# simplify23/TPS_PP

Hardware: AMD Instinct MI355X
Metric: rectified images/sec (3x32x100) (higher is better)
Workload: dtype f32; 1 GPU; BASELINE.json configs[1]: fused TPS grid-gen + bilinear grid_sample HIP kernel, batch 512 per GPU, 3x32x100 fp32, 20 fiducials, inputs resident in HBM; batch_per_gpu=512, rotating_buffer_sets=14, streams=3, repeats=1

## Files before the change

### tps_pp_amd/csrc/tpspp_warp_pair.h

```cpp
#pragma once
#include "tpspp_warp_dev.h"

namespace tpspp_pair {

using namespace tpspp_dev;

typedef float v4f __attribute__((ext_vector_type(4)));
typedef float v4f_a4 __attribute__((ext_vector_type(4), aligned(4)));
typedef __attribute__((address_space(1))) char gchar;

struct PairParams {
    const float* in; const float* ctrl; const float* inv_delta_c;
    const float* packed;
    const float* p_hat;
    int p_hat_ld;
    int N;
    float* out; float* grid; int32_t* idx;
    int zero_off;
    int out_off;
    long long* trace;
};

template <int F>
__device__ __forceinline__ constexpr int perm_y(int k) { return (k + F / 2) % F; }
template <int F>
__device__ __forceinline__ constexpr int perm_x(int k) { return k < F / 2 ? F / 2 - 1 - k : F + F / 2 - 1 - k; }

__device__ __forceinline__ void store16_nt(gchar* p, v4f v)
{
    asm volatile("global_store_dwordx4 %0, %1, off nt\n\ts_nop 1" ::"v"(p), "v"(v) : "memory");
}

__device__ __forceinline__ void wait_flag(const float* flag_word, int want)
{
    const volatile int* f = reinterpret_cast<const volatile int*>(flag_word);
    while (*f < want) __builtin_amdgcn_s_sleep(1);
}
__device__ __forceinline__ void wait_flag_lds(const float* flag_word, int want)
{
    typedef __attribute__((address_space(3))) const volatile int lds_cvint;
    lds_cvint* f = (lds_cvint*)(size_t)(unsigned)(size_t)flag_word;
    while (__builtin_amdgcn_readfirstlane(*f) < want) __builtin_amdgcn_s_sleep(1);
}

template <int OFF>
__device__ __forceinline__ void flag_add(unsigned addr, int one)
{
    asm volatile("ds_add_u32 %0, %1 offset:%2" ::"v"(addr), "v"(one), "n"(OFF) : "memory");
}

struct TapsLite {
    int o00;
    float nw, ne, sw, se;
    float wx, wy;
    bool inx, iny;
    int x0, y0;
};
__device__ __forceinline__ TapsLite make_taps_lite(float gx, float gy, int H, int W)
{
    TapsLite t;
    const float limx = (float)(W - 1), limy = (float)(H - 1);
    float ix = (gx + 1.0f) * (0.5f * limx);
    float iy = (gy + 1.0f) * (0.5f * limy);
    ix = (ix > 0.0f) ? ix : 0.0f;
    iy = (iy > 0.0f) ? iy : 0.0f;
    ix = __builtin_fminf(ix, limx);
    iy = __builtin_fminf(iy, limy);
    const float w = __builtin_amdgcn_fractf(ix), nn = __builtin_amdgcn_fractf(iy);
    int x0, y0;
    asm("v_cvt_flr_i32_f32 %0, %1" : "=v"(x0) : "v"(ix));
    asm("v_cvt_flr_i32_f32 %0, %1" : "=v"(y0) : "v"(iy));
    const float e = 1.0f - w, s = 1.0f - nn;
    t.nw = s * e; t.ne = s * w; t.sw = nn * e; t.se = nn * w;
    t.wx = w; t.wy = nn;
    t.inx = ix < limx;
    t.iny = iy < limy;
    t.o00 = __mul24(y0, W) + x0;
    t.x0 = x0; t.y0 = y0;
    return t;
}

constexpr int kPairFlags = 4;
constexpr int kPairLoaders = 3;
constexpr int kPairAwait = 6;
constexpr int kPairKB = 4;

constexpr int kPairVarPacked = 1;
constexpr int kPairVarMfma = 2;
typedef float v2f __attribute__((ext_vector_type(2)));

template <int OH, int OW>
struct PairGeo {
    static constexpr int halfW = OW / 2;
    static constexpr int PW = (halfW + 3) & ~3;
    static constexpr int CGP = PW / 4;
    static constexpr int CG = (halfW - 2) / 4;
    static constexpr int SC0 = CG * 4;
    static constexpr int SW = OW - 2 * SC0;
    static constexpr int nthr = (OH / 2) * CG * 4;
    static constexpr int NW = nthr / kWave;
    static_assert(OW % 4 == 0 && (OH / 2) % 8 == 0 && nthr % kWave == 0, "needs whole 4 x 8 pixel blocks, whole wavefronts");
    static_assert(SW == 4 && OH * SW == 2 * kWave, "the centre strip is 4 columns, two wavefronts per image");
    static_assert(NW % 4 == 0 && NW >= 4, "the compute wavefronts spread evenly over the four SIMDs");
};
__host__ __device__ inline void pair_thread_pixel(int t, int CG, int* r, int* c)
{
    const int hw = t >> 5, l5 = t & 31, rg = hw / CG, cg = hw - rg * CG;
    *r = rg * 8 + (l5 >> 2);
    *c = cg * 4 + (l5 & 3);
}

template <int F, int C, int HC, int WC, int OH, int OW, bool AUX, bool TRACE, int VAR = 0>
__global__ void __launch_bounds__(1024)
tps_warp_pair_kernel(const PairParams P)
{
    using Geo = PairGeo<OH, OW>;
    constexpr int K = F + 3;
    constexpr int H = HC, W = WC;
    constexpr int NW = Geo::NW, NLOAD = kPairLoaders;
    constexpr int n = OH * OW;
    static_assert(NW + NLOAD <= 16, "too many wavefronts");
    extern __shared__ __attribute__((aligned(16))) float smem[];
    float4* sT = reinterpret_cast<float4*>(smem);
    float* sFlag = smem + 4 * K + 2 * ((K * K + 3) & ~3);
    float* sImg = sFlag + kPairFlags;
    float* sZero = sImg + P.zero_off;
    float* sOut = sImg + P.out_off;

    const int tid = threadIdx.x;
    const int lane = tid & (kWave - 1);
    const int wv = __builtin_amdgcn_readfirstlane(tid / kWave);
    const int b0 = blockIdx.x * 2;
    const bool hasB = (b0 + 1) < P.N;
    constexpr int HW = H * W;
    constexpr int img_elems = C * HW;

    unsigned ts[8];
#define PAIR_STAMP(i) do { if (TRACE) ts[i] = (unsigned)__builtin_amdgcn_s_memtime(); } while (0)
    long long wall0 = 0;
    if (TRACE) wall0 = (long long)wall_clock64();
    PAIR_STAMP(7);

    constexpr int KGI = (K + 3) / 4;
    float hrowv[KGI * 4];
    float cx = 0.0f, cy = 0.0f;
    if (wv < 2) {
        if (lane < F) {
            const int b = (wv == 1 && hasB) ? b0 + 1 : b0;
            const float2 cc = reinterpret_cast<const float2*>(P.ctrl + (size_t)b * F * 2)[lane];
            cx = cc.x; cy = cc.y;
        }
        const float* row = P.inv_delta_c + (lane < K ? lane : K - 1) * K;
#pragma unroll
        for (int j = 0; j < KGI; ++j) {
            const int c0 = (j == KGI - 1) ? K - 4 : 4 * j;
            const v4f_a4 x = *reinterpret_cast<const v4f_a4*>(row + c0);
            hrowv[4 * j] = x[0]; hrowv[4 * j + 1] = x[1]; hrowv[4 * j + 2] = x[2]; hrowv[4 * j + 3] = x[3];
        }
    }
    if (tid < kPairFlags) reinterpret_cast<int*>(sFlag)[tid] = 0;
    lds_only_barrier();

    if (wv >= NW) {
        const int lw = wv - NW;
        const int total_bytes = (hasB ? 2 : 1) * img_elems * 4;
        const int pieces = (total_bytes + 1023) >> 10;
        const int piecesA = (img_elems * 4 + 1023) >> 10;
        const char* src = reinterpret_cast<const char*>(P.in + (size_t)b0 * img_elems);
        auto dma = [&](int piece) {
            int off = piece * 1024 + lane * 16;
            if (off >= total_bytes) off = 0;
            __builtin_amdgcn_global_load_lds(
                (const __attribute__((address_space(1))) void*)(src + off),
                (__attribute__((address_space(3))) void*)(reinterpret_cast<char*>(sImg) + piece * 1024),
                16, 0, 2 );
        };
        unsigned fa = (unsigned)(size_t)(sFlag + 1), fb = (unsigned)(size_t)(sFlag + 2);
        int one = 1;
        asm volatile("" : "+v"(fa), "+v"(fb), "+v"(one));
        int piece = lw;
        for (; piece < piecesA; piece += NLOAD) dma(piece);
        asm volatile("s_waitcnt vmcnt(%0)" ::"n"(kPairAwait) : "memory");
#pragma unroll
        for (int i = 0; i < kPairKB; ++i) { if (piece < pieces) dma(piece); piece += NLOAD; }
        if (hasB) asm volatile("s_waitcnt vmcnt(%0)" ::"n"(kPairKB) : "memory");
        else      asm volatile("s_waitcnt vmcnt(0)" ::: "memory");
        if (lane == 0) flag_add<0>(fa, one);
        for (; piece < pieces; piece += NLOAD) dma(piece);
        asm volatile("s_waitcnt vmcnt(0)" ::: "memory");
        if (lane == 0) flag_add<0>(fb, one);
        return;
    }

    const int hw = tid >> 5, l5 = tid & 31;
    const int rg = hw / Geo::CG, cg = hw - rg * Geo::CG;
    const int r = rg * 8 + (l5 >> 2), c = cg * 4 + (l5 & 3);
    unsigned poff[4];
    poff[0] = 4u * (unsigned)(r * OW + c);
    poff[1] = 4u * (unsigned)(r * OW + (OW - 1 - c));
    poff[2] = 4u * (unsigned)((OH - 1 - r) * OW + c);
    poff[3] = 4u * (unsigned)((OH - 1 - r) * OW + (OW - 1 - c));
    const bool strip = wv < 4 && (wv < 2 || hasB);
    const int sim = wv >> 1;
    const int srow = (wv & 1) * (OH / 2) + (lane >> 2), scol = Geo::SC0 + (lane & 3);
    const unsigned spoff = 4u * (unsigned)(srow * OW + scol);

    constexpr int KG = (K + 3) / 4;
    float v[KG * 4];
    {
        const int t_old = (rg * Geo::CGP + cg) * 32 + l5;
        const v4f* pk = reinterpret_cast<const v4f*>(P.packed) + (size_t)(t_old >> 6) * KG * kWave + (t_old & (kWave - 1));
#pragma unroll
        for (int j = 0; j < KG; ++j) {
            const v4f x = pk[j * kWave];
            v[4 * j] = x[0]; v[4 * j + 1] = x[1]; v[4 * j + 2] = x[2]; v[4 * j + 3] = x[3];
        }
    }
    float u[KG * 4];
    if (wv < 4) {
        const float* row = P.p_hat + (size_t)(srow * OW + scol) * P.p_hat_ld;
#pragma unroll
        for (int j = 0; j < KG; ++j) {
            const v4f_a4 x = *reinterpret_cast<const v4f_a4*>(row + 4 * j);
            u[4 * j] = x[0]; u[4 * j + 1] = x[1]; u[4 * j + 2] = x[2]; u[4 * j + 3] = x[3];
        }
    }
    if (tid < C) sZero[tid * HW] = 0.0f;
    if (wv < 2) {
        float ax = 0.0f, ay = 0.0f;
        static_for<K>([&](auto qc) {
            constexpr int q = decltype(qc)::value;
            constexpr int idx = (q / 4 < KGI - 1) ? q : 4 * (KGI - 1) + (q - (K - 4));
            ax = fmaf(hrowv[idx], readlane_f(cx, q), ax);
            ay = fmaf(hrowv[idx], readlane_f(cy, q), ay);
        });
        if (lane < K) {
            float* dst = reinterpret_cast<float*>(sT + lane) + 2 * wv;
            dst[0] = ax; dst[1] = ay;
        }
        asm volatile("s_waitcnt lgkmcnt(0)" ::: "memory");
        if (lane == 0) __hip_atomic_fetch_add(reinterpret_cast<int*>(sFlag), 1, __ATOMIC_RELAXED, __HIP_MEMORY_SCOPE_WORKGROUP);
    }
    wait_flag_lds(sFlag + 0, 2);
    PAIR_STAMP(0);
    asm volatile("" ::"v"(v[KG * 4 - 1]), "v"(u[KG * 4 - 1]));

    float sgx = 0.0f, sgy = 0.0f;
    if (wv < 4) {
        static_for<K>([&](auto qc) {
            constexpr int q = decltype(qc)::value;
            const float2 t = reinterpret_cast<const float2*>(sT + q)[sim];
            sgx = fmaf(u[q], t.x, sgx);
            sgy = fmaf(u[q], t.y, sgy);
        });
        asm volatile("" : "+v"(sgx), "+v"(sgy));
    }

    float gx[4][2], gy[4][2];
#pragma unroll
    for (int m = 0; m < 4; ++m) gx[m][0] = gx[m][1] = gy[m][0] = gy[m][1] = 0.0f;
    if constexpr ((VAR & kPairVarMfma) != 0) {
        v4f macc[4];
#pragma unroll
        for (int m = 0; m < 4; ++m) macc[m] = v4f{0.0f, 0.0f, 0.0f, 0.0f};
        const float* tcomp = reinterpret_cast<const float*>(sT) + (lane & 3);
        static_for<K>([&](auto qc) {
            constexpr int q = decltype(qc)::value;
            const float tq = tcomp[4 * q];
            float val[4];
            if constexpr (q == 0) {
                val[0] = val[1] = val[2] = val[3] = v[0];
            } else if constexpr (q == 1) {
                val[0] = v[1]; val[1] = -v[1]; val[2] = v[1]; val[3] = -v[1];
            } else if constexpr (q == 2) {
                val[0] = v[2]; val[1] = v[2]; val[2] = -v[2]; val[3] = -v[2];
            } else {
                constexpr int k = q - 3;
                val[0] = v[3 + k];
                val[1] = v[3 + perm_x<F>(k)];
                val[2] = v[3 + perm_y<F>(k)];
                val[3] = v[3 + perm_x<F>(perm_y<F>(k))];
            }
#pragma unroll
            for (int m = 0; m < 4; ++m) macc[m] = __builtin_amdgcn_mfma_f32_4x4x1f32(tq, val[m], macc[m], 0, 0, 0);
        });
#pragma unroll
        for (int m = 0; m < 4; ++m) { gx[m][0] = macc[m][0]; gy[m][0] = macc[m][1]; gx[m][1] = macc[m][2]; gy[m][1] = macc[m][3]; }
    } else
    static_for<K>([&](auto qc) {
        constexpr int q = decltype(qc)::value;
        const float4 t = sT[q];
        float val[4];
        if constexpr (q == 0) {
            val[0] = val[1] = val[2] = val[3] = v[0];
        } else if constexpr (q == 1) {
            val[0] = v[1]; val[1] = -v[1]; val[2] = v[1]; val[3] = -v[1];
        } else if constexpr (q == 2) {
            val[0] = v[2]; val[1] = v[2]; val[2] = -v[2]; val[3] = -v[2];
        } else {
            constexpr int k = q - 3;
            val[0] = v[3 + k];
            val[1] = v[3 + perm_x<F>(k)];
            val[2] = v[3 + perm_y<F>(k)];
            val[3] = v[3 + perm_x<F>(perm_y<F>(k))];
        }
        if constexpr (VAR & kPairVarPacked) {
            const v2f tA = {t.x, t.y}, tB = {t.z, t.w};
#pragma unroll
            for (int m = 0; m < 4; ++m) {
                const v2f vv = {val[m], val[m]};
                v2f a = {gx[m][0], gy[m][0]}, b = {gx[m][1], gy[m][1]};
                a = __builtin_elementwise_fma(vv, tA, a);
                b = __builtin_elementwise_fma(vv, tB, b);
                gx[m][0] = a.x; gy[m][0] = a.y; gx[m][1] = b.x; gy[m][1] = b.y;
            }
        } else {
#pragma unroll
            for (int m = 0; m < 4; ++m) {
                gx[m][0] = fmaf(val[m], t.x, gx[m][0]);
                gy[m][0] = fmaf(val[m], t.y, gy[m][0]);
                gx[m][1] = fmaf(val[m], t.z, gx[m][1]);
                gy[m][1] = fmaf(val[m], t.w, gy[m][1]);
            }
        }
    });
#pragma unroll
    for (int m = 0; m < 4; ++m) asm volatile("" : "+v"(gx[m][0]), "+v"(gy[m][0]), "+v"(gx[m][1]), "+v"(gy[m][1]));

    constexpr unsigned row_bytes = n * 4u;
    constexpr int out16 = (C * n) >> 2;
    constexpr int nct = NW * kWave;
    typedef __attribute__((address_space(3))) const float lds_cfloat;
    const unsigned img_lds = (unsigned)(size_t)sImg, zero_lds = (unsigned)(size_t)sZero;
    auto describe_px = [&](float pgx, float pgy, int im, unsigned pix_off, bool st, unsigned (&a)[4], float (&w)[4]) {
        const TapsLite t = make_taps_lite(pgx, pgy, H, W);
        if constexpr (AUX) {
            const int b = b0 + im;
            if (P.grid && st)
                *reinterpret_cast<float2*>(reinterpret_cast<char*>(P.grid) + (size_t)b * 2 * row_bytes + 2u * pix_off) = make_float2(pgx, pgy);
            if (P.idx && st)
                *reinterpret_cast<int2*>(reinterpret_cast<char*>(P.idx) + (size_t)b * 2 * row_bytes + 2u * pix_off) = make_int2(t.x0, t.y0);
        }
        const unsigned a0 = img_lds + (unsigned)(im * img_elems * 4) + 4u * (unsigned)t.o00;
        a[0] = a0;
        a[1] = t.inx ? a0 + 4u : zero_lds;
        a[2] = t.iny ? a0 + 4u * W : zero_lds;
        a[3] = (t.inx && t.iny) ? a0 + 4u * W + 4u : zero_lds;
        w[0] = t.nw; w[1] = t.ne; w[2] = t.sw; w[3] = t.se;
    };
    unsigned ta[2][4][4];
    float tw[2][4][4];
#pragma unroll
    for (int im = 0; im < 2; ++im) {
#pragma unroll
        for (int m = 0; m < 4; ++m) describe_px(gx[m][im], gy[m][im], im, poff[m], im == 0 || hasB, ta[im][m], tw[im][m]);
#pragma unroll
        for (int m = 0; m < 4; ++m)
#pragma unroll
            for (int q = 0; q < 4; ++q) asm volatile("" : "+v"(ta[im][m][q]), "+v"(tw[im][m][q]));
    }
    unsigned sa[4] = {zero_lds, zero_lds, zero_lds, zero_lds};
    float sw[4] = {0.0f, 0.0f, 0.0f, 0.0f};
    if (wv < 4) describe_px(sgx, sgy, sim, spoff, strip, sa, sw);
    PAIR_STAMP(1);

    constexpr int NOUT = (out16 + nct - 1) / nct;
    v4f ostage[NOUT];
    auto store_image = [&](int b) {
        gchar* ob = (gchar*)(P.out) + (size_t)b * C * row_bytes;
#pragma unroll
        for (int i = 0; i < NOUT; ++i) {
            const int e = tid + i * nct;
            if (e < out16) store16_nt(ob + 16u * (unsigned)e, ostage[i]);
        }
    };
    auto read_staged = [&](const float* stage) {
#pragma unroll
        for (int i = 0; i < NOUT; ++i) {
            const int e = tid + i * nct;
            if (e < out16) ostage[i] = *reinterpret_cast<const v4f*>(reinterpret_cast<const char*>(stage) + 16 * e);
        }
    };
    auto load_taps = [&](int im, float (&tv)[4][C][4]) {
#pragma unroll
        for (int m = 0; m < 4; ++m)
#pragma unroll
            for (int ch = 0; ch < C; ++ch)
#pragma unroll
                for (int q = 0; q < 4; ++q) tv[m][ch][q] = *((lds_cfloat*)(size_t)(ta[im][m][q]) + ch * HW);
    };
    auto finish_image = [&](auto barc, int im, float (&tv)[4][C][4], bool mystrip, float* stage) {
        constexpr bool BAR = decltype(barc)::value;
        float res[4][C], sres[C];
#pragma unroll
        for (int m = 0; m < 4; ++m)
#pragma unroll
            for (int ch = 0; ch < C; ++ch) {
                float acc = tv[m][ch][0] * tw[im][m][0];
                acc = fmaf(tv[m][ch][1], tw[im][m][1], acc);
                acc = fmaf(tv[m][ch][2], tw[im][m][2], acc);
                acc = fmaf(tv[m][ch][3], tw[im][m][3], acc);
                res[m][ch] = acc;
            }
        if (mystrip) {
            __builtin_amdgcn_sched_barrier(0);
            float sv[C][4];
#pragma unroll
            for (int ch = 0; ch < C; ++ch)
#pragma unroll
                for (int q = 0; q < 4; ++q) sv[ch][q] = *((lds_cfloat*)(size_t)(sa[q]) + ch * HW);
#pragma unroll
            for (int ch = 0; ch < C; ++ch) {
                float acc = sv[ch][0] * sw[0];
                acc = fmaf(sv[ch][1], sw[1], acc);
                acc = fmaf(sv[ch][2], sw[2], acc);
                acc = fmaf(sv[ch][3], sw[3], acc);
                sres[ch] = acc;
            }
        }
        if (BAR) lds_only_barrier();
#pragma unroll
        for (int m = 0; m < 4; ++m)
#pragma unroll
            for (int ch = 0; ch < C; ++ch)
                *reinterpret_cast<float*>(reinterpret_cast<char*>(stage) + ch * (int)row_bytes + poff[m]) = res[m][ch];
        if (mystrip) {
#pragma unroll
            for (int ch = 0; ch < C; ++ch)
                *reinterpret_cast<float*>(reinterpret_cast<char*>(stage) + ch * (int)row_bytes + spoff) = sres[ch];
        }
    };

#pragma unroll
    for (int im = 0; im < 2; ++im) {
        if (im == 1 && !hasB) { store_image(b0); break; }
        wait_flag_lds(sFlag + 1 + im, NLOAD);
        PAIR_STAMP(2 + 2 * im);
        float tv[4][C][4];
        load_taps(im, tv);
        if (im == 1) {
            __builtin_amdgcn_sched_barrier(0);
            store_image(b0);
            __builtin_amdgcn_sched_barrier(0);
            finish_image(std::true_type{}, im, tv, strip && sim == im, sOut);
        } else {
            finish_image(std::false_type{}, im, tv, strip && sim == im, sOut);
        }
        lds_only_barrier();
        PAIR_STAMP(3 + 2 * im);
        read_staged(sOut);
        if (im == 1) {
            store_image(b0 + 1);
        } else {
            asm volatile("s_waitcnt lgkmcnt(0)" ::: "memory");
#pragma unroll
            for (int i = 0; i < NOUT; ++i) asm volatile("" : "+v"(ostage[i]));
        }
    }
    if (TRACE && wv == 0) {
        asm volatile("s_waitcnt vmcnt(0)" ::: "memory");
        PAIR_STAMP(6);
        if (lane == 0 && P.trace) {
            long long* t = P.trace + (size_t)blockIdx.x * 8;
            if (!hasB) ts[4] = ts[5] = ts[3];
#pragma unroll
            for (int i = 0; i < 7; ++i) t[i] = (long long)(ts[i] - ts[7]);
            t[7] = wall0;
        }
    }
#undef PAIR_STAMP
}


template <int F, int C, int HC, int WC, int OH, int OW>
inline size_t pair_lds_bytes(int* zero_off, int* out_off)
{
    constexpr int K = F + 3;
    const int pieces = (2 * C * HC * WC * 4 + 1023) / 1024;
    *zero_off = pieces * 256;
    *out_off = pieces * 256 + (C - 1) * HC * WC + 4;
    return (size_t)(4 * K + 2 * ((K * K + 3) & ~3) + kPairFlags) * sizeof(float) + (size_t)(*out_off) * 4 + (size_t)C * OH * OW * 4;
}

}
```

Measured before the change: 63.38 million images/s.

## Interleave channels 0 and 1 in LDS so each bilinear tap reads a float2

Adds a template variant where the loader wavefronts use 4-byte global_load_lds requests to interleave channels 0 and 1 of each image into pairs in LDS, with channel 2 copied as a plain plane. Tap gathers then do one 8-byte LDS read for channels 0-1 plus one 4-byte read for channel 2, replacing three scalar reads. The zero-word addresses and wait counts are adjusted to match, and there are tunable await, prefetch and loader-count knobs. The trade is many more, smaller DMA requests to build the interleaved layout, in exchange for fewer LDS gather instructions. The path only runs when VAR selects it.

After: 62.68 million images/s. 1.1% lower.

```diff
diff --git a/tps_pp_amd/csrc/tpspp_warp_pair.h b/tps_pp_amd/csrc/tpspp_warp_pair.h
--- a/tps_pp_amd/csrc/tpspp_warp_pair.h
+++ b/tps_pp_amd/csrc/tpspp_warp_pair.h
@@ -88,6 +88,12 @@
 constexpr int kPairVarPacked = 1;
 constexpr int kPairVarMfma = 2;
 typedef float v2f __attribute__((ext_vector_type(2)));
+constexpr int kPairVarInterleave = 4;
+constexpr int kPairVarLoad4 = 8;
+constexpr int kPairVarTuneShift = 4;
+constexpr int pair_il_await(int var) { const int t[4] = {24, 12, 24, 6}; return t[(var >> kPairVarTuneShift) & 3]; }
+constexpr int pair_il_kb(int var)    { const int t[4] = {16, 8, 4, 4};   return t[(var >> kPairVarTuneShift) & 3]; }
+constexpr int pair_loaders(int var) { return (var & kPairVarLoad4) ? 4 : kPairLoaders; }
 
 template <int OH, int OW>
 struct PairGeo {
@@ -117,7 +123,8 @@
     using Geo = PairGeo<OH, OW>;
     constexpr int K = F + 3;
     constexpr int H = HC, W = WC;
-    constexpr int NW = Geo::NW, NLOAD = kPairLoaders;
+    constexpr int NW = Geo::NW, NLOAD = pair_loaders(VAR);
+    constexpr bool IL = (VAR & kPairVarInterleave) != 0 && C == 3;
     constexpr int n = OH * OW;
     static_assert(NW + NLOAD <= 16, "too many wavefronts");
     extern __shared__ __attribute__((aligned(16))) float smem[];
@@ -163,6 +170,50 @@
 
     if (wv >= NW) {
         const int lw = wv - NW;
+        if constexpr (IL) {
+            constexpr int plane_b = HW * 4;
+            static_assert(HW % 32 == 0, "whole 256-byte requests");
+            constexpr int RP = 2 * plane_b / 256, RC = (plane_b + 1023) / 1024, R = RP + RC;
+            constexpr int AW = pair_il_await(VAR), KB = pair_il_kb(VAR);
+            static_assert(KB <= R / NLOAD, "every loader issues KB of image B's requests in front of flag A");
+            static_assert(AW + (R + NLOAD - 1) / NLOAD <= 63, "vmcnt is a 6-bit counter");
+            const char* src = reinterpret_cast<const char*>(P.in + (size_t)b0 * img_elems);
+            const int lane_pair = (lane & 1) * plane_b + (lane >> 1) * 4;
+            const int lane_c2 = lane * 16;
+            auto dma = [&](int im, int rq) {
+                const char* s = src + im * (img_elems * 4);
+                char* d = reinterpret_cast<char*>(sImg) + im * (img_elems * 4);
+                if (rq < RP) {
+                    __builtin_amdgcn_global_load_lds(
+                        (const __attribute__((address_space(1))) void*)(s + rq * 128 + lane_pair),
+                        (__attribute__((address_space(3))) void*)(d + rq * 256), 4, 0, 2 );
+                } else {
+                    const int k = rq - RP;
+                    if (k * 1024 + lane_c2 < plane_b)
+                        __builtin_amdgcn_global_load_lds(
+                            (const __attribute__((address_space(1))) void*)(s + 2 * plane_b + k * 1024 + lane_c2),
+                            (__attribute__((address_space(3))) void*)(d + 2 * plane_b + k * 1024), 16, 0, 2 );
+                }
+            };
+            unsigned fa = (unsigned)(size_t)(sFlag + 1), fb = (unsigned)(size_t)(sFlag + 2);
+            int one = 1;
+            asm volatile("" : "+v"(fa), "+v"(fb), "+v"(one));
+            for (int rq = lw; rq < R; rq += NLOAD) dma(0, rq);
+            asm volatile("s_waitcnt vmcnt(%0)" ::"n"(AW) : "memory");
+            int rq = lw;
+            if (hasB) {
+#pragma unroll
+                for (int i = 0; i < KB; ++i) { dma(1, rq); rq += NLOAD; }
+                asm volatile("s_waitcnt vmcnt(%0)" ::"n"(KB) : "memory");
+            } else {
+                asm volatile("s_waitcnt vmcnt(0)" ::: "memory");
+            }
+            if (lane == 0) flag_add<0>(fa, one);
+            if (hasB) for (; rq < R; rq += NLOAD) dma(1, rq);
+            asm volatile("s_waitcnt vmcnt(0)" ::: "memory");
+            if (lane == 0) flag_add<0>(fb, one);
+            return;
+        }
         const int total_bytes = (hasB ? 2 : 1) * img_elems * 4;
         const int pieces = (total_bytes + 1023) >> 10;
         const int piecesA = (img_elems * 4 + 1023) >> 10;
@@ -225,6 +276,10 @@
             u[4 * j] = x[0]; u[4 * j + 1] = x[1]; u[4 * j + 2] = x[2]; u[4 * j + 3] = x[3];
         }
     }
+    if constexpr (IL) {
+        static_assert(HW % 2 == 0, "image B's zero word is 1.5 planes behind image A's");
+        if (tid < 4) sZero[tid == 0 ? 0 : tid == 1 ? 3 * HW / 2 : 2 * HW + (tid - 2)] = 0.0f;
+    } else
     if (tid < C) sZero[tid * HW] = 0.0f;
     if (wv < 2) {
         float ax = 0.0f, ay = 0.0f;
@@ -331,7 +386,11 @@
     constexpr int out16 = (C * n) >> 2;
     constexpr int nct = NW * kWave;
     typedef __attribute__((address_space(3))) const float lds_cfloat;
+    typedef __attribute__((address_space(3))) const v2f lds_cv2f;
     const unsigned img_lds = (unsigned)(size_t)sImg, zero_lds = (unsigned)(size_t)sZero;
+    auto il_c2 = [&](int im) { return img_lds + (unsigned)(im * img_elems * 4) + 8u * HW; };
+    auto il_zero = [&](int im) { return zero_lds + (im ? 6u * HW : 0u); };
+    auto il_k = [&](int im) { return (img_lds + (unsigned)(im * img_elems * 4)) - 2u * il_c2(im); };
     auto describe_px = [&](float pgx, float pgy, int im, unsigned pix_off, bool st, unsigned (&a)[4], float (&w)[4]) {
         const TapsLite t = make_taps_lite(pgx, pgy, H, W);
         if constexpr (AUX) {
@@ -341,11 +400,12 @@
             if (P.idx && st)
                 *reinterpret_cast<int2*>(reinterpret_cast<char*>(P.idx) + (size_t)b * 2 * row_bytes + 2u * pix_off) = make_int2(t.x0, t.y0);
         }
-        const unsigned a0 = img_lds + (unsigned)(im * img_elems * 4) + 4u * (unsigned)t.o00;
+        const unsigned a0 = (IL ? il_c2(im) : img_lds + (unsigned)(im * img_elems * 4)) + 4u * (unsigned)t.o00;
+        const unsigned az = IL ? il_zero(im) : zero_lds;
         a[0] = a0;
-        a[1] = t.inx ? a0 + 4u : zero_lds;
-        a[2] = t.iny ? a0 + 4u * W : zero_lds;
-        a[3] = (t.inx && t.iny) ? a0 + 4u * W + 4u : zero_lds;
+        a[1] = t.inx ? a0 + 4u : az;
+        a[2] = t.iny ? a0 + 4u * W : az;
+        a[3] = (t.inx && t.iny) ? a0 + 4u * W + 4u : az;
         w[0] = t.nw; w[1] = t.ne; w[2] = t.sw; w[3] = t.se;
     };
     unsigned ta[2][4][4];
@@ -387,7 +447,18 @@
 #pragma unroll
             for (int ch = 0; ch < C; ++ch)
 #pragma unroll
-                for (int q = 0; q < 4; ++q) tv[m][ch][q] = *((lds_cfloat*)(size_t)(ta[im][m][q]) + ch * HW);
+                for (int q = 0; q < 4; ++q) {
+                    if constexpr (IL) {
+                        if (ch == 0) {
+                            const v2f p01 = *(lds_cv2f*)(size_t)(2u * ta[im][m][q] + il_k(im));
+                            tv[m][0][q] = p01.x; tv[m][1][q] = p01.y;
+                        } else if (ch == 2) {
+                            tv[m][2][q] = *(lds_cfloat*)(size_t)(ta[im][m][q]);
+                        }
+                    } else {
+                        tv[m][ch][q] = *((lds_cfloat*)(size_t)(ta[im][m][q]) + ch * HW);
+                    }
+                }
     };
     auto finish_image = [&](auto barc, int im, float (&tv)[4][C][4], bool mystrip, float* stage) {
         constexpr bool BAR = decltype(barc)::value;
@@ -408,7 +479,18 @@
 #pragma unroll
             for (int ch = 0; ch < C; ++ch)
 #pragma unroll
-                for (int q = 0; q < 4; ++q) sv[ch][q] = *((lds_cfloat*)(size_t)(sa[q]) + ch * HW);
+                for (int q = 0; q < 4; ++q) {
+                    if constexpr (IL) {
+                        if (ch == 0) {
+                            const v2f p01 = *(lds_cv2f*)(size_t)(2u * sa[q] + il_k(sim));
+                            sv[0][q] = p01.x; sv[1][q] = p01.y;
+                        } else if (ch == 2) {
+                            sv[2][q] = *(lds_cfloat*)(size_t)(sa[q]);
+                        }
+                    } else {
+                        sv[ch][q] = *((lds_cfloat*)(size_t)(sa[q]) + ch * HW);
+                    }
+                }
 #pragma unroll
             for (int ch = 0; ch < C; ++ch) {
                 float acc = sv[ch][0] * sw[0];
```
